# aikiriao/AAD

Hardware: AMD Instinct MI355X
Metric: Msamples/s encode+decode, 48 kHz stereo 4-bit (higher is better)
Workload: dtype int32

## Files before the change

### aad_amd/capi.py

```python
import ctypes as C
import os

import numpy as np


class AADApiResult:
    OK = 0
    INVALID_ARGUMENT = 1
    INVALID_FORMAT = 2
    INSUFFICIENT_BUFFER = 3
    INSUFFICIENT_DATA = 4
    PARAMETER_NOT_SET = 5
    NG = 6
    _names = {0: "OK", 1: "INVALID_ARGUMENT", 2: "INVALID_FORMAT", 3: "INSUFFICIENT_BUFFER",
              4: "INSUFFICIENT_DATA", 5: "PARAMETER_NOT_SET", 6: "NG"}

    @classmethod
    def name(cls, v):
        return cls._names.get(int(v), str(v))


class AADHeaderInfo(C.Structure):
    _fields_ = [("format_version", C.c_uint32), ("codec_version", C.c_uint32),
                ("num_channels", C.c_uint16), ("num_samples", C.c_uint32),
# ... 48 lines not shown

STREAM_DESC_DTYPE = np.dtype([("pcm_offset", "<u8"), ("data_offset", "<u8"), ("data_size", "<u8"),
                              ("num_samples", "<u4"), ("reserved", "<u4")])
ERROR_STATS_DTYPE = np.dtype([("rms_error", "<f8"), ("mean_abs_error", "<f8"), ("max_abs_error", "<f8")])
WINDOW_DTYPE = np.dtype([("stream", "<i8"), ("first_frame", "<i8")])
SAMPLE_INT16, SAMPLE_FLOAT32 = 0, 1
SAMPLE_FLOAT16, SAMPLE_BFLOAT16 = 4, 5
RESAMPLE_NO_BANK = 0xFFFF
WINDOW_GAIN_STORE, WINDOW_GAIN_ADD = 0, 1
RECONSTRUCT_DECODED, RECONSTRUCT_RESIDUAL = 0, 1
OPTION_LANE_MAPPING, OPTION_TRIAL_LANES, OPTION_STAGING_THREADS, OPTION_TILE_KBYTES, OPTION_COMPARE_ORDER = 0, 1, 2, 3, 4
LANE_MAPPINGS = {"auto": 0, "dense": 1, "quad": 2, "quad-fused": 3, "dense-tiled": 4}
TRIAL_LANES = {"dual": 0, "single": 1}
OPTION_SIMD_ROLE = 5
SIMD_ROLE_OFF = -1
LANE_STATE_DTYPE = np.dtype([("weight", "<i4", (4,)), ("history", "<i4", (4,)),
                             ("stepsize_index", "<i4"), ("quantize_error", "<i4")])

_PKG_DIR = os.path.dirname(os.path.abspath(__file__))
LIBRARY_PATH = os.environ.get("AAD_HIP_LIBRARY", os.path.join(_PKG_DIR, "libaad_hip.so"))

LEGACY_SYMBOLS = [
    "AADEncoder_CalculateBlockSize", "AADEncoder_EncodeHeader", "AADEncoder_CalculateWorkSize",
    "AADEncoder_Create", "AADEncoder_Destroy", "AADEncoder_SetEncodeParameter", "AADEncoder_EncodeWhole",
    "AADDecoder_DecodeHeader", "AADDecoder_CalculateWorkSize", "AADDecoder_Create", "AADDecoder_Destroy",
    "AADDecoder_SetHeader", "AADDecoder_DecodeBlock", "AADDecoder_DecodeWhole",
]
HIP_SYMBOLS = [
    "AADHip_GetDeviceCount", "AADHip_ContextCreate", "AADHip_ContextDestroy", "AADHip_ContextSynchronize",
    "AADHip_ContextLastError", "AADHip_ContextSignalNextRun", "AADHip_SignalNextRunSupported", "AADHip_ContextSetOption", "AADHip_CalculateEncodedSize", "AADHip_EncodePlanCreate",
    "AADHip_EncodePlanDestroy", "AADHip_EncodePlanRun", "AADHip_DecodePlanCreate", "AADHip_DecodePlanDestroy",
    "AADHip_DecodePlanRun", "AADHip_EncodeBatch", "AADHip_DecodeBatch",
    "AADHip_ReconstructPlanCreate", "AADHip_ReconstructPlanDestroy", "AADHip_ReconstructPlanRun",
    "AADHip_ReconstructBatch", "AADHip_SegmentedEncodePlanCreate", "AADHip_SegmentedEncodeBatch",
    "AADHip_SegmentedReconstructPlanCreate", "AADHip_SegmentedReconstructBatch",
    "AADHip_WindowDecodePlanCreate", "AADHip_WindowDecodePlanDestroy", "AADHip_WindowDecodePlanRun",
    "AADHip_WindowDecodePlanRunStats", "AADHip_WindowDecodePlanRunGain", "AADHip_WindowDecodePlanRunPlaced", "AADHip_WindowDecodePlanRunPlacedStats",
    "AADHip_MixedWindowDecodePlanCreate", "AADHip_ChannelMixWindowDecodePlanCreate",
    "AADHip_PlanarEncodePlanCreate", "AADHip_PlanarEncodePlanRun",
    "AADHip_PlanarReconstructPlanCreate", "AADHip_PlanarReconstructPlanRun", "AADHip_PlanarReconstructPlanRunStats",
    "AADHip_WindowReconstructPlanCreate", "AADHip_WindowReconstructPlanDestroy", "AADHip_WindowReconstructPlanRun",
    "AADHip_ResamplerCreate", "AADHip_ResamplerDestroy", "AADHip_ResamplerBank", "AADHip_ResamplerSourceFrames",
    "AADHip_ResamplerResolve", "AADHip_ResamplerRun", "AADHip_ResamplerRunGain", "AADHip_ResamplerRunStats",
    "AADHip_ResamplerCreateWide",
]
WAV_SYMBOLS = ["AADWav_ParseHeader", "AADWav_WriteHeader", "AADWav_ConvertToPcm16"]
SYNTH_SYMBOLS = ["AADSynth_Generate"]


class AADWavInfo(C.Structure):
    _fields_ = [("format_tag", C.c_uint16), ("num_channels", C.c_uint16), ("sampling_rate", C.c_uint32),
                ("bits_per_sample", C.c_uint16), ("num_samples", C.c_uint32), ("data_offset", C.c_uint64),
                ("data_size", C.c_uint64)]


def _declare_legacy(lib):
    u8p, i32pp = C.POINTER(C.c_uint8), C.POINTER(C.POINTER(C.c_int32))
    lib.AADEncoder_CalculateBlockSize.argtypes = [C.c_uint16, C.c_uint16, C.c_uint32,
                                                  C.POINTER(C.c_uint16), C.POINTER(C.c_uint32)]
# ... 65 lines not shown
    lib.AADHip_PlanarReconstructPlanRun.restype = C.c_int
    lib.AADHip_PlanarReconstructPlanRunStats.argtypes = [vp, vp, vp, vp, vp, vp]
    lib.AADHip_PlanarReconstructPlanRunStats.restype = C.c_int
    lib.AADHip_WindowReconstructPlanCreate.argtypes = [vp, C.POINTER(AADEncodeParameter), C.POINTER(AADHipPlanarLayout),
                                                       C.POINTER(AADHipSegmentation), C.c_uint32, vp, C.POINTER(vp)]
    lib.AADHip_WindowReconstructPlanCreate.restype = C.c_int
    lib.AADHip_WindowReconstructPlanDestroy.argtypes = [vp]
    lib.AADHip_WindowReconstructPlanDestroy.restype = None
    lib.AADHip_WindowReconstructPlanRun.argtypes = [vp, vp, C.c_uint64, vp, C.c_uint32, C.c_uint64, vp, C.POINTER(AADHipPlanarOutput),
                                                    vp, vp]
    lib.AADHip_WindowReconstructPlanRun.restype = C.c_int
    lib.AADHip_EncodePlanDestroy.argtypes = [vp]
    lib.AADHip_EncodePlanDestroy.restype = None
    lib.AADHip_EncodePlanRun.argtypes = [vp, vp, vp, vp]
    lib.AADHip_EncodePlanRun.restype = C.c_int
    lib.AADHip_DecodePlanCreate.argtypes = [vp, C.POINTER(AADHeaderInfo), C.c_int32, C.c_uint32, vp, C.POINTER(vp)]
    lib.AADHip_DecodePlanCreate.restype = C.c_int
    lib.AADHip_DecodePlanDestroy.argtypes = [vp]
    lib.AADHip_DecodePlanDestroy.restype = None
    lib.AADHip_DecodePlanRun.argtypes = [vp, vp, vp]
    lib.AADHip_DecodePlanRun.restype = C.c_int
    lib.AADHip_WindowDecodePlanCreate.argtypes = [vp, C.POINTER(AADHeaderInfo), C.c_int32, C.c_uint32, vp, C.POINTER(vp)]
    lib.AADHip_WindowDecodePlanCreate.restype = C.c_int
    lib.AADHip_MixedWindowDecodePlanCreate.argtypes = [vp, C.c_uint32, C.c_int32, C.c_uint32, vp, vp, C.POINTER(vp)]
    lib.AADHip_MixedWindowDecodePlanCreate.restype = C.c_int
    lib.AADHip_ChannelMixWindowDecodePlanCreate.argtypes = [vp, C.c_uint32, C.c_int32, C.c_uint32, vp, vp, C.POINTER(vp)]
    lib.AADHip_ChannelMixWindowDecodePlanCreate.restype = C.c_int
    lib.AADHip_WindowDecodePlanDestroy.argtypes = [vp]
    lib.AADHip_WindowDecodePlanDestroy.restype = None
    lib.AADHip_WindowDecodePlanRun.argtypes = [vp, vp, C.c_uint64, vp, C.c_uint32, C.c_int32, vp]
# ... 169 lines not shown
```

### aad_amd/csrc/aad_encode.hip.h

```cpp
#ifndef AAD_ENCODE_HIP_H
#define AAD_ENCODE_HIP_H

#include "aad_device.hip.h"
#include "aad_pcm_convert.h"
#include "aad_segments.h"

namespace aad {

constexpr bool kEncTM = true;

template <int BITS>
__device__ __forceinline__ int32_t index_delta_arith(uint32_t mag)
{
  if (BITS == 4) {
    const uint32_t corr = __builtin_amdgcn_perm(0u, 0x00161514u, mag) & 0xFFu;
    return (int32_t)(2u << mag) - (int32_t)corr;
  } else if (BITS == 3) {
    return mag < 2 ? (int32_t)mag - 16 : (int32_t)(2u << (2u * mag));
  } else {
    return mag ? 40 : -14;
  }
}

template <int BITS>
// ... 1864 lines not shown
  if constexpr (rec_has_stats(REC)) {
    if constexpr (SEG) rec.template finish<true>(a.stats + (uint64_t)a.stats_stream[s] * ch + c, total - warm_end);
    else rec.template finish<false>(a.stats + lane, total > a.lead_frames ? total - a.lead_frames : 0u);
  }

  if (!SEG && a.state_out && writer) {
    LaneStateRecord r;
    r.weight[0] = F.w0; r.weight[1] = F.w1; r.weight[2] = F.w2; r.weight[3] = F.w3;
    r.history[0] = F.h0; r.history[1] = F.h1; r.history[2] = F.h2; r.history[3] = F.h3;
    r.stepsize_index = F.idxb - kIdxBias;
    r.quantize_error = last_qd;
    a.state_out[lane] = r;
  }
}

}

#endif
```

### aad_amd/csrc/aad_encode_launch.hip.h

```cpp
#ifndef AAD_ENCODE_LAUNCH_HIP_H
#define AAD_ENCODE_LAUNCH_HIP_H

#include "aad_encode.hip.h"
#include "aad_launch.h"

namespace aad {

template <int BITS, bool QUAD, bool TRIALS, bool DUAL, bool RING = false, bool SEG = false, int IN = kInInterleaved, int REC = kRecNone>
void launch_encode_mapped(const KernelArgsFor<IN, REC> &a, const EncodeLaunch &p, hipStream_t stream)
{
  const dim3 grid(p.grid), block(p.workgroup);
  if (a.channels == 1) {
    if constexpr (IN != kInPlanarI16)
      AAD_LAUNCH((encode_streams_kernel<BITS, 1, false, QUAD, TRIALS, DUAL, RING, SEG, IN, REC>), grid, block, p.lds, stream, a);
  } else if constexpr (IN == kInInterleaved && REC != kRecNone) {
  } else if (a.channels == 2 && a.mid_side)
    AAD_LAUNCH((encode_streams_kernel<BITS, 2, true, QUAD, TRIALS, DUAL, RING, SEG, IN, REC>), grid, block, p.lds, stream, a);
  else if (a.channels == 2)
    AAD_LAUNCH((encode_streams_kernel<BITS, 2, false, QUAD, TRIALS, DUAL, RING, SEG, IN, REC>), grid, block, p.lds, stream, a);
  else if constexpr (!QUAD && !RING)
    AAD_LAUNCH((encode_streams_kernel<BITS, 0, false, false, TRIALS, false, false, SEG, IN, REC>), grid, block, p.lds, stream, a);
}

template <int BITS, bool SEG, int IN = kInInterleaved, int REC = kRecNone>
// ... 50 lines not shown
    a.stats = r.stats;
    a.stats_stream = r.stats_stream;
  }
  auto by_bits = [&](auto seg) {
    constexpr bool SEG = decltype(seg)::value;
    switch (a.bits) {
      case 4: launch_encode<4, SEG, IN, REC>(a, p, stream); break;
      case 3: launch_encode<3, SEG, IN, REC>(a, p, stream); break;
      default: launch_encode<2, SEG, IN, REC>(a, p, stream); break;
    }
  };
  if (r.chain_table) by_bits(std::true_type{});
  else by_bits(std::false_type{});
}

extern template void launch_encode_run<kInPlanarI16, kRecNone>(const EncodeRun &, const EncodeLaunch &, hipStream_t);
extern template void launch_encode_run<kInPlanarF32, kRecNone>(const EncodeRun &, const EncodeLaunch &, hipStream_t);
#define AAD_EXTERN_REC_RUN(REC)                                                                                    \
  extern template void launch_encode_run<kInInterleaved, REC>(const EncodeRun &, const EncodeLaunch &, hipStream_t); \
  extern template void launch_encode_run<kInPlanarI16, REC>(const EncodeRun &, const EncodeLaunch &, hipStream_t);   \
  extern template void launch_encode_run<kInPlanarF32, REC>(const EncodeRun &, const EncodeLaunch &, hipStream_t);
AAD_EXTERN_REC_RUN(kRecI16)
AAD_EXTERN_REC_RUN(kRecF32)
AAD_EXTERN_REC_RUN(kRecI16Stats)
AAD_EXTERN_REC_RUN(kRecF32Stats)
AAD_EXTERN_REC_RUN(kRecStatsOnly)
#undef AAD_EXTERN_REC_RUN

}

// ... 2 lines not shown
```

### aad_amd/csrc/aad_hip_engine.hip

```cpp
#include <hip/hip_runtime.h>

#include <cstdio>
#include <cstdlib>
#include <cstring>
#include <algorithm>
#include <condition_variable>
#include <functional>
#include <mutex>
#include <new>
#include <thread>
#include <vector>

#include "../../include/aad_hip.h"
#include "aad_compare.hip.h"
#include "aad_launch.h"
#include "aad_decode.hip.h"
#include "aad_decode_window.hip.h"
#include "aad_decode_window_mixed.hip.h"
#include "aad_decode_window_channel_mix.hip.h"
#include "aad_encode.hip.h"
#include "aad_encode_launch.hip.h"
#include "aad_format.h"
#include "aad_hip_internal.h"
#include "aad_resample.hip.h"
#include "aad_tiles.h"
#include "aad_window_reconstruct.hip.h"

namespace aad {
thread_local LaunchSignal tl_launch_signal = {nullptr, nullptr};
}

static_assert(sizeof(AADHipStreamDesc) == sizeof(aad::StreamDesc), "stream table layout");
static_assert(sizeof(AADHipLaneState) == sizeof(aad::LaneStateRecord), "lane state layout");
static_assert(sizeof(AADHipErrorStats) == sizeof(aad::ErrorStatsRecord), "error stats layout");

struct Staging {
  void *host = nullptr, *dev = nullptr;
  size_t cap = 0;
};

struct StagingPool {
  std::vector<std::thread> threads;
  std::mutex lock;
  std::condition_variable work, done;
// ... 48 lines not shown
  AADHipStreamDesc *d_sources;
  uint32_t num_sources;
  uint8_t *d_lanes;
  uint64_t lanes_capacity;
};

struct AADHipEncodePlan {
  AADHipContext *ctx;
  EncodePlanKind kind;
  aad::EncodeRun run;
  void *d_table;
  uint64_t *d_out_base;
  uint32_t *d_stats_stream;
  uint64_t stats_records;
  WindowPlanPart *windows;
};

struct AADHipDecodePlan {
  AADHipContext *ctx;
  aad::DecodeArgs args;
  aad::StreamDesc *d_streams;
  uint64_t *d_prefix;
};

struct AADHipWindowDecodePlan {
  AADHipContext *ctx;
  aad::DecodeArgs args;
  aad::StreamDesc *d_streams;
  bool mixed;
  aad::StreamFormat *d_formats;
// ... 356 lines not shown
  }
  if (output != nullptr && !aad::planar_output_ok(args.channels, num_streams, streams, output)) {
    snprintf(ctx->last_error, sizeof(ctx->last_error),
             "planar reconstruct plan: output rows refused (sample type, reserved, a stride below the rows, or past 64-bit offsets)");
    return AAD_APIRESULT_INVALID_ARGUMENT;
  }
  AADHipEncodePlan *p = new (std::nothrow) AADHipEncodePlan();
  if (p == nullptr) return AAD_APIRESULT_NG;
  p->ctx = ctx;
  p->kind = output != nullptr ? EncodePlanKind::Reconstruct : (layout != nullptr ? EncodePlanKind::Rows : EncodePlanKind::Frames);
  p->d_table = nullptr;
  p->d_out_base = nullptr;
  p->d_stats_stream = nullptr;
  p->windows = nullptr;
  p->stats_records = (uint64_t)num_streams * args.channels;
  DeviceGuard guard(ctx);
  bool ok = guard.ok;
  if (ok && segmentation != nullptr) {
    aad::ChainDesc *d_chains = nullptr;
    ok = upload(ctx, &d_chains, chains.data(), chains.size());
    p->d_table = d_chains;
    use_chain_table(&run, d_chains, (uint32_t)chains.size());
  } else if (ok) {
    aad::StreamDesc *d_streams = nullptr;
    ok = upload(ctx, &d_streams, reinterpret_cast<const aad::StreamDesc *>(streams), num_streams);
    p->d_table = d_streams;
    run.args.streams = d_streams;
  }
  if (ok && output != nullptr) {
    const std::vector<uint64_t> base =
// ... 214 lines not shown
const char *AADHip_ContextLastError(const struct AADHipContext *ctx) { return ctx ? ctx->last_error : ""; }

void AADHipInternal_ContextOptionsFromEnvironment(struct AADHipContext *ctx)
{
  static const char *const kMappings[] = {"auto", "dense", "quad", "quad-fused", "dense-tiled"};
  static const char *const kTrialLanes[] = {"dual", "single"};
  ctx->signal_refused = AADHip_SignalNextRunSupported() == 0;
  ctx->knobs.lane_mapping = option_from_env("AAD_HIP_MAPPING", kMappings, 5);
  ctx->knobs.trial_lanes = option_from_env("AAD_HIP_TRIAL_LANES", kTrialLanes, 2);
  const char *ring = getenv("AAD_HIP_ENCODE_RING"), *enc_pad = getenv("AAD_HIP_ENCODE_LDS_PAD");
  const char *dec_pad = getenv("AAD_HIP_DECODE_LDS_PAD"), *nt_min = getenv("AAD_HIP_DECODE_NT_MIN");
  ctx->knobs.encode_ring = ring != nullptr && ring[0] == '0' ? 0 : (ring != nullptr && ring[0] == '2' ? 2 : 1);
  ctx->knobs.encode_lds_pad = enc_pad ? atoi(enc_pad) : -1;
  ctx->knobs.decode_lds_pad = dec_pad ? atoi(dec_pad) : -1;
  ctx->knobs.decode_nt_min = nt_min ? (uint64_t)atoll(nt_min) : 0ull;
  static const char *const kCompareOrders[] = {"auto", "sequential"};
  ctx->compare_sequential = option_from_env("AAD_HIP_COMPARE_ORDER", kCompareOrders, 2);
  const char *threads = getenv("AAD_HIP_STAGING_THREADS");
  if (threads != nullptr && threads[0] >= '1' && threads[0] <= '8' && threads[1] == '\0') ctx->staging_threads = threads[0] - '0';
  const char *tile = getenv("AAD_HIP_TILE_KBYTES");
  if (tile != nullptr) {
    const long long v = atoll(tile);
    if (v > 0 && v <= 0x7FFFFFFF) ctx->tile_bytes = (int64_t)v << 10;
  }
}

int32_t AADHipInternal_ContextDevice(const struct AADHipContext *ctx) { return ctx->device; }

int32_t AADHip_SignalNextRunSupported(void)
{
// ... 17 lines not shown
AADApiResult AADHip_ContextSetOption(struct AADHipContext *ctx, int32_t option, int32_t value)
{
  if (ctx == nullptr) return AAD_APIRESULT_INVALID_ARGUMENT;
  switch (option) {
    case AAD_HIP_OPTION_LANE_MAPPING:
      if (value < AAD_HIP_LANE_MAPPING_AUTO || value > AAD_HIP_LANE_MAPPING_DENSE_TILED) return AAD_APIRESULT_INVALID_ARGUMENT;
      ctx->knobs.lane_mapping = value;
      return AAD_APIRESULT_OK;
    case AAD_HIP_OPTION_TRIAL_LANES:
      if (value != AAD_HIP_TRIAL_LANES_DUAL && value != AAD_HIP_TRIAL_LANES_SINGLE) return AAD_APIRESULT_INVALID_ARGUMENT;
      ctx->knobs.trial_lanes = value;
      return AAD_APIRESULT_OK;
    case AAD_HIP_OPTION_SIMD_ROLE:
      if (value < AAD_HIP_SIMD_ROLE_OFF || value > AAD_HIP_SIMD_ROLE_3) return AAD_APIRESULT_INVALID_ARGUMENT;
      ctx->knobs.simd_role = value;
      return AAD_APIRESULT_OK;
    case AAD_HIP_OPTION_COMPARE_ORDER:
      if (value != 0 && value != 1) return AAD_APIRESULT_INVALID_ARGUMENT;
      ctx->compare_sequential = value;
      return AAD_APIRESULT_OK;
    case AAD_HIP_OPTION_STAGING_THREADS:
      if (value < 0 || value > 8) return AAD_APIRESULT_INVALID_ARGUMENT;
      ctx->staging_threads = value;
      return AAD_APIRESULT_OK;
    case AAD_HIP_OPTION_TILE_KBYTES:
      if (value < 0) return AAD_APIRESULT_INVALID_ARGUMENT;
      ctx->tile_bytes = (int64_t)value << 10;
      return AAD_APIRESULT_OK;
    default:
      return AAD_APIRESULT_INVALID_ARGUMENT;
// ... 41 lines not shown
AADApiResult AADHip_SegmentedEncodePlanCreate(struct AADHipContext *ctx, const struct AADEncodeParameter *parameter,
                                              const struct AADHipSegmentation *segmentation, uint32_t num_streams,
                                              const struct AADHipStreamDesc *streams, struct AADHipEncodePlan **plan)
{
  if (ctx == nullptr || parameter == nullptr || segmentation == nullptr || plan == nullptr || (num_streams != 0 && streams == nullptr))
    return AAD_APIRESULT_INVALID_ARGUMENT;
  *plan = nullptr;
  if (segmentation->segment_blocks == 0) return AAD_APIRESULT_INVALID_ARGUMENT;
  return encode_plan_create(ctx, parameter, nullptr, nullptr, segmentation, num_streams, streams, plan);
}

AADApiResult AADHip_EncodePlanRun(struct AADHipEncodePlan *plan, const int16_t *device_pcm, uint8_t *device_data,
                                  struct AADHipLaneState *device_state)
{
  return encode_plan_run(plan, EncodePlanKind::Frames, device_pcm, device_data, nullptr, device_state);
}


AADApiResult AADHip_PlanarEncodePlanCreate(struct AADHipContext *ctx, const struct AADEncodeParameter *parameter,
                                           const struct AADHipPlanarLayout *layout, const struct AADHipSegmentation *segmentation,
                                           uint32_t num_streams, const struct AADHipStreamDesc *streams, struct AADHipEncodePlan **plan)
{
  if (ctx == nullptr || parameter == nullptr || layout == nullptr || plan == nullptr || (num_streams != 0 && streams == nullptr))
    return AAD_APIRESULT_INVALID_ARGUMENT;
  *plan = nullptr;
  if (!planar_fields_ok(layout, segmentation)) return AAD_APIRESULT_INVALID_ARGUMENT;
  return encode_plan_create(ctx, parameter, layout, nullptr, segmentation, num_streams, streams, plan);
}

AADApiResult AADHip_PlanarEncodePlanRun(struct AADHipEncodePlan *plan, const void *device_samples, uint8_t *device_data,
// ... 1876 lines not shown
```

### aad_amd/csrc/aad_launch_policy.h

```cpp
#ifndef AAD_LAUNCH_POLICY_H
#define AAD_LAUNCH_POLICY_H

#include <stdint.h>

#include "../../include/aad_hip.h"
#include "aad_lds_layout.h"

namespace aad {

struct Device {
  uint32_t cus, lds_per_cu;
};

struct Knobs {
  int32_t lane_mapping = AAD_HIP_LANE_MAPPING_AUTO;
  int32_t trial_lanes = AAD_HIP_TRIAL_LANES_DUAL;
  int32_t encode_ring = 1;
  int32_t encode_lds_pad = -1;
  int32_t decode_lds_pad = -1;
  uint64_t decode_nt_min = 0;
  int32_t simd_role = AAD_HIP_SIMD_ROLE_OFF;
};

struct EncodeBatch {
  uint32_t bits, channels, streams, trials, block_size;
  bool ring_ok;
};

struct DecodeBatch {
  uint64_t blocks;
  uint32_t streams, channels, bits, samples_per_block, block_size, code_phase_uniform;
  bool pcm_aligned16, pcm_base_aligned16, stream_stores;
};

enum class EncodeKernel { Dense, DenseRing, Quad, QuadDual };
struct EncodeLaunch {
// ... 86 lines not shown
    }
    return p;
  }
  p.kernel = EncodeKernel::Dense;
  uint32_t static_lds = dense_encoder_lds(b.bits, b.channels);
  p.workgroup = dense_encode_workgroup(d, lanes, static_lds);
  p.grid = grid_for(lanes, p.workgroup);
  if (p.trials) return p;
  if (b.ring_ok && b.channels <= 2 && encode_ring_wanted(k, b.bits, b.channels, p.workgroup)) {
    p.kernel = EncodeKernel::DenseRing;
    p.lds = (p.workgroup / 64u) * (uint32_t)(b.channels == 1 ? kLdsRingBytesPerWave<1> : kLdsRingBytesPerWave<2>);
    static_lds = (uint32_t)kLdsCodeStageOff + p.lds;
  }
  if (p.workgroup == 256u) p.lds += dense_encode_lds_pad(d, k, b.bits, lanes, static_lds);
  return p;
}

inline EncodeLaunch plan_reconstruct_encode(const Device &d, const Knobs &k, const EncodeBatch &b)
{
  Knobs r = k;
  r.trial_lanes = AAD_HIP_TRIAL_LANES_SINGLE;
  r.encode_ring = 0;
  return plan_encode(d, r, b);
}

inline bool planar_output_rows_ok(uint32_t channels, uint64_t num_streams, uint64_t longest, const AADHipPlanarOutput *o)
{
  if (o == nullptr || channels == 0) return false;
  if ((o->sample_type != AAD_HIP_SAMPLE_INT16 && o->sample_type != AAD_HIP_SAMPLE_FLOAT32) || o->reserved != 0) return false;
  if (channels > 1 && o->channel_stride < longest) return false;
// ... 297 lines not shown
```

### aad_amd/engine.py

```python
import ctypes as C
from collections import namedtuple

import numpy as np

from .capi import (AADApiResult, AADHeaderInfo, AADHipResampleRatio, RESAMPLE_NO_BANK, AADHipPlanarLayout, AADHipPlanarOutput, AADHipSegmentation, ApiError, ERROR_STATS_DTYPE, LANE_MAPPINGS, LANE_STATE_DTYPE,
                   OPTION_COMPARE_ORDER, OPTION_LANE_MAPPING, OPTION_SIMD_ROLE, OPTION_STAGING_THREADS, OPTION_TILE_KBYTES, OPTION_TRIAL_LANES, RECONSTRUCT_DECODED, RECONSTRUCT_RESIDUAL,
                   SAMPLE_BFLOAT16, SAMPLE_FLOAT16, SAMPLE_FLOAT32, SAMPLE_INT16, SIMD_ROLE_OFF, STREAM_DESC_DTYPE, TRIAL_LANES, WINDOW_DTYPE, WINDOW_GAIN_ADD, WINDOW_GAIN_STORE, load_library, make_parameter)


def _check(where, rc):
    if rc != AADApiResult.OK:
        raise ApiError(where, rc)


def _round_up(v, a):
    return (v + a - 1) // a * a


def tensor_span(t):
    if any(int(s) == 0 for s in t.shape):
        return 0
    return 1 + sum((int(s) - 1) * int(st) for s, st in zip(t.shape, t.stride()))


# ... 159 lines not shown
        _check("AADHip_ContextSetOption",
               self.lib.AADHip_ContextSetOption(self._ctx, OPTION_STAGING_THREADS, int(threads)))

    def set_tile_kbytes(self, kbytes=0):
        _check("AADHip_ContextSetOption",
               self.lib.AADHip_ContextSetOption(self._ctx, OPTION_TILE_KBYTES, int(kbytes)))

    def set_compare_order(self, sequential=False):
        _check("AADHip_ContextSetOption",
               self.lib.AADHip_ContextSetOption(self._ctx, OPTION_COMPARE_ORDER, 1 if sequential else 0))

    def set_simd_role(self, simd=None):
        _check("AADHip_ContextSetOption",
               self.lib.AADHip_ContextSetOption(self._ctx, OPTION_SIMD_ROLE, SIMD_ROLE_OFF if simd is None else int(simd)))

    def synchronize(self):
        _check("AADHip_ContextSynchronize", self.lib.AADHip_ContextSynchronize(self._ctx))

    def encoded_size(self, param, num_samples):
        return int(self.lib.AADHip_CalculateEncodedSize(C.byref(param), num_samples))

    def encode_plan(self, param, descs, segment_blocks=None, warmup_blocks=0):
        descs = np.ascontiguousarray(descs, dtype=STREAM_DESC_DTYPE)
        plan = C.c_void_p()
        if segment_blocks is None:
            _check("AADHip_EncodePlanCreate",
                   self.lib.AADHip_EncodePlanCreate(self._ctx, C.byref(param), len(descs), descs.ctypes.data, C.byref(plan)))
        else:
            seg = AADHipSegmentation(int(segment_blocks), int(warmup_blocks))
            _check("AADHip_SegmentedEncodePlanCreate",
# ... 617 lines not shown
        return self._extents[kind]

    def run(self, pcm, data, state=None, ordered=True):
        if state is not None and self.segmented:
            raise ValueError("a segmented encode plan takes no state")
        e = self.engine
        e.tensor("pcm", pcm, e.torch.int16, self.extent("interleaved"), rows_in_place=True, memo=self._memo)
        e.tensor("data", data, e.torch.uint8, self.extent("images"), rows_in_place=True, memo=self._memo)
        e.state_tensor(state, len(self.descs), self.param.num_channels, self._memo)
        sp = state.data_ptr() if state is not None else None
        cur = self.engine._enter() if ordered else None
        _check("AADHip_EncodePlanRun",
               self.engine.lib.AADHip_EncodePlanRun(self.handle, pcm.data_ptr(), data.data_ptr(), sp))
        if ordered:
            self.engine._exit(cur)

    def close(self):
        if self.handle:
            self.engine.lib.AADHip_EncodePlanDestroy(self.handle)
            self.handle = None

    def __del__(self):
        try:
            self.close()
        except Exception:
            pass


class PlanarEncodePlan(EncodePlan):
    def __init__(self, engine, handle, param, descs, dtype, channel_stride):
# ... 489 lines not shown
        assert enc_engine.stream.cuda_stream != dec_engine.stream.cuda_stream, "the two contexts need streams of their own"
        torch = enc_engine.torch
        self.torch, self.ring, self.k = torch, ring, 0
        self.enc_engine, self.dec_engine = enc_engine, dec_engine
        self._take_simd_roles(_simd_roles.setdefault(enc_engine.device, SimdRoleAllocator()) if simd_roles else None)
        self.enc = enc_engine.uniform_encode_plan(param, streams, samples)
        self.images = [torch.zeros((streams, self.enc.stride), dtype=torch.uint8, device="cuda:%d" % enc_engine.device)
                       for _ in range(ring)]
        zero = torch.zeros((streams, samples, param.num_channels), dtype=torch.int16, device=self.images[0].device)
        self.enc.run(zero, self.images[0])
        torch.cuda.synchronize()
        self.header = parse_header(bytes(self.images[0][0, :31].cpu().numpy()))
        self.dec = dec_engine.uniform_decode_plan(self.header, streams, self.images[0].stride(0), self.enc.image_size)
        self.encoded = [HipEvent() for _ in range(ring)]
        self.decoded = [torch.cuda.Event() for _ in range(ring)]

    def step(self, pcm, out, timing=None):
        k, ring = self.k, self.ring
        self.k += 1
        b = k % ring
        s_enc, s_dec = self.enc_engine.stream, self.dec_engine.stream
        if k >= ring and k % (ring // 2) == 0:
            s_enc.wait_event(self.decoded[(k - ring // 2 - 1) % ring])
        encoded = self.encoded[b] if timing is None else timing[1]
        self.enc_engine.signal_next(encoded, start=None if timing is None else timing[0])
        self.enc.run(pcm, self.images[b], None, ordered=False)
        encoded.wait_on(s_dec)
        if timing is not None:
            self.dec_engine.signal_next(timing[3], start=timing[2])
        self.dec.run(self.images[b], out, ordered=False)
        self.decoded[b].record(s_dec)
        return self.images[b]

    def close(self):
        self.torch.cuda.synchronize()
        self.enc.close()
        self.dec.close()
        for e in self.encoded:
            e.close()
        self._release_simd_roles()

    def _take_simd_roles(self, allocator):
        self._roles = allocator
        self._role_slot = allocator.acquire(self._set_simd_roles) if allocator is not None else None

    def _set_simd_roles(self, enc_simd, dec_simd):
        self.enc_engine.set_simd_role(enc_simd)
        self.dec_engine.set_simd_role(dec_simd)

    def _release_simd_roles(self):
        if getattr(self, "_role_slot", None) is not None:
            self._roles.release(self._role_slot)
            self._role_slot = None


def parse_header(data):
    if len(data) < 31 or data[:4] != b"AAD\x00":
        raise ApiError("parse_header", AADApiResult.INVALID_FORMAT)
    be = lambda o, n: int.from_bytes(data[o:o + n], "big")
    return AADHeaderInfo(format_version=be(4, 4), codec_version=be(8, 4), num_channels=be(12, 2),
                         num_samples=be(14, 4), sampling_rate=be(18, 4), bits_per_sample=be(22, 2),
                         block_size=be(24, 2), num_samples_per_block=be(26, 4), ch_process_method=data[30])

# ... 3 lines not shown
```

### include/aad_hip.h

```cpp
#ifndef AAD_HIP_H_INCLUDED
#define AAD_HIP_H_INCLUDED

#include <stdint.h>
#include "aad.h"
#include "aad_encoder.h"

#define AAD_HIP_MAX_NUM_CHANNELS 8

struct AADHipContext;
struct AADHipEncodePlan;
struct AADHipDecodePlan;

struct AADHipStreamDesc {
  uint64_t pcm_offset;
  uint64_t data_offset;
  uint64_t data_size;
  uint32_t num_samples;
  uint32_t reserved;
};

struct AADHipLaneState {
  int32_t weight[4];
  int32_t history[4];
  int32_t stepsize_index;
// ... 8 lines not shown

AADApiResult AADHip_ContextCreate(int32_t device_index, void *hip_stream, struct AADHipContext **context);
void AADHip_ContextDestroy(struct AADHipContext *context);
AADApiResult AADHip_ContextSynchronize(struct AADHipContext *context);
const char *AADHip_ContextLastError(const struct AADHipContext *context);

AADApiResult AADHip_ContextSignalNextRun(struct AADHipContext *context, void *hip_start_event, void *hip_stop_event);
int32_t AADHip_SignalNextRunSupported(void);

enum AADHipOption {
  AAD_HIP_OPTION_LANE_MAPPING = 0,
  AAD_HIP_OPTION_TRIAL_LANES = 1,
  AAD_HIP_OPTION_STAGING_THREADS = 2,
  AAD_HIP_OPTION_TILE_KBYTES = 3,
  AAD_HIP_OPTION_COMPARE_ORDER = 4,
  AAD_HIP_OPTION_SIMD_ROLE = 5
};
enum AADHipSimdRole {
  AAD_HIP_SIMD_ROLE_OFF = -1,
  AAD_HIP_SIMD_ROLE_0 = 0, AAD_HIP_SIMD_ROLE_1 = 1, AAD_HIP_SIMD_ROLE_2 = 2, AAD_HIP_SIMD_ROLE_3 = 3
};
enum AADHipLaneMapping {
  AAD_HIP_LANE_MAPPING_AUTO = 0,
  AAD_HIP_LANE_MAPPING_DENSE = 1,
  AAD_HIP_LANE_MAPPING_QUAD = 2,
  AAD_HIP_LANE_MAPPING_QUAD_FUSED = 3,
  AAD_HIP_LANE_MAPPING_DENSE_TILED = 4
};
enum AADHipTrialLanes {
  AAD_HIP_TRIAL_LANES_DUAL = 0,
  AAD_HIP_TRIAL_LANES_SINGLE = 1
};
AADApiResult AADHip_ContextSetOption(struct AADHipContext *context, int32_t option, int32_t value);

uint64_t AADHip_CalculateEncodedSize(const struct AADEncodeParameter *parameter, uint32_t num_samples);


AADApiResult AADHip_EncodePlanCreate(
    struct AADHipContext *context, const struct AADEncodeParameter *parameter,
    uint32_t num_streams, const struct AADHipStreamDesc *streams,
    struct AADHipEncodePlan **plan);
void AADHip_EncodePlanDestroy(struct AADHipEncodePlan *plan);

AADApiResult AADHip_EncodePlanRun(
    struct AADHipEncodePlan *plan, const int16_t *device_pcm, uint8_t *device_data,
    struct AADHipLaneState *device_state);


struct AADHipSegmentation {
  uint32_t segment_blocks;
  uint32_t warmup_blocks;
};
AADApiResult AADHip_SegmentedEncodePlanCreate(
    struct AADHipContext *context, const struct AADEncodeParameter *parameter,
    const struct AADHipSegmentation *segmentation,
    uint32_t num_streams, const struct AADHipStreamDesc *streams,
    struct AADHipEncodePlan **plan);


AADApiResult AADHip_DecodePlanCreate(
    struct AADHipContext *context, const struct AADHeaderInfo *format, int32_t has_file_header,
// ... 251 lines not shown
```

Measured before the change: 122,100.

## Split pipeline encode into resumable spans so decode overlaps encode tail

Adds a span-encode kernel that resumes from saved lane state at chunk-aligned frames. The encode+decode pipeline now encodes the first ~95% of frames, signals the decoder's stream, then encodes the remainder on the decoder's stream (roles off by default). The intent is to let the decoder's stream start earlier and shorten the cross-stream dependency. It adds a second launch, state records that must be zeroed each ring half, and extra synchronisation when the split is first enabled.

```diff
diff --git a/aad_amd/capi.py b/aad_amd/capi.py
--- a/aad_amd/capi.py
+++ b/aad_amd/capi.py
@@ -86,6 +86,7 @@
 TRIAL_LANES = {"dual": 0, "single": 1}
 OPTION_SIMD_ROLE = 5
 SIMD_ROLE_OFF = -1
+OPTION_PIPELINE_SPLIT = 6
 LANE_STATE_DTYPE = np.dtype([("weight", "<i4", (4,)), ("history", "<i4", (4,)),
                              ("stepsize_index", "<i4"), ("quantize_error", "<i4")])
 
@@ -115,6 +116,7 @@
     "AADHip_ResamplerCreate", "AADHip_ResamplerDestroy", "AADHip_ResamplerBank", "AADHip_ResamplerSourceFrames",
     "AADHip_ResamplerResolve", "AADHip_ResamplerRun", "AADHip_ResamplerRunGain", "AADHip_ResamplerRunStats",
     "AADHip_ResamplerCreateWide",
+    "AADHip_EncodePlanRunSpan", "AADHip_EncodePlanSpanSupported", "AADHip_EncodePlanSpanFloor", "AADHip_EncodePlanPipelineSplit",
 ]
 WAV_SYMBOLS = ["AADWav_ParseHeader", "AADWav_WriteHeader", "AADWav_ConvertToPcm16"]
 SYNTH_SYMBOLS = ["AADSynth_Generate"]
@@ -210,6 +212,14 @@
     lib.AADHip_EncodePlanDestroy.restype = None
     lib.AADHip_EncodePlanRun.argtypes = [vp, vp, vp, vp]
     lib.AADHip_EncodePlanRun.restype = C.c_int
+    lib.AADHip_EncodePlanRunSpan.argtypes = [vp, vp, vp, vp, C.c_uint32, C.c_uint32]
+    lib.AADHip_EncodePlanRunSpan.restype = C.c_int
+    lib.AADHip_EncodePlanSpanSupported.argtypes = [vp]
+    lib.AADHip_EncodePlanSpanSupported.restype = C.c_int32
+    lib.AADHip_EncodePlanSpanFloor.argtypes = [vp, C.c_uint32]
+    lib.AADHip_EncodePlanSpanFloor.restype = C.c_uint32
+    lib.AADHip_EncodePlanPipelineSplit.argtypes = [vp, C.c_int32]
+    lib.AADHip_EncodePlanPipelineSplit.restype = C.c_uint32
     lib.AADHip_DecodePlanCreate.argtypes = [vp, C.POINTER(AADHeaderInfo), C.c_int32, C.c_uint32, vp, C.POINTER(vp)]
     lib.AADHip_DecodePlanCreate.restype = C.c_int
     lib.AADHip_DecodePlanDestroy.argtypes = [vp]
diff --git a/aad_amd/csrc/aad_encode.hip.h b/aad_amd/csrc/aad_encode.hip.h
--- a/aad_amd/csrc/aad_encode.hip.h
+++ b/aad_amd/csrc/aad_encode.hip.h
@@ -2,6 +2,7 @@
 #define AAD_ENCODE_HIP_H
 
 #include "aad_device.hip.h"
+#include "aad_encode_span.h"
 #include "aad_pcm_convert.h"
 #include "aad_segments.h"
 
@@ -1902,6 +1903,85 @@
   }
 }
 
+
+struct SpanEncodeArgs : EncodeArgs {
+  uint32_t first_frame, frame_count;
+};
+static_assert(kSpanSeedFrames == (uint32_t)kTaps && kSpanChunkFrames == (uint32_t)kChunk, "aad_encode_span.h counts in the kernels' units");
+
+template <int BITS, int CHF, bool MS>
+__global__ void __launch_bounds__(256) encode_span_kernel(SpanEncodeArgs a)
+{
+  static_assert(CHF == 1 || CHF == 2, "the quad mapping: mono / stereo");
+  __shared__ __attribute__((aligned(16))) char lds[kLdsBytesEncoderStatic<BITS, CHF, true, false>];
+  __shared__ uint32_t s_wave_simd[4];
+  if (a.simd_role) publish_wave_simd(s_wave_simd);
+  stage_tables<BITS, true, kWideStepShift, true>(lds);
+  uint64_t thread = (uint64_t)blockIdx.x * blockDim.x + threadIdx.x;
+  if (a.simd_role) {
+    if ((threadIdx.x >> 6) != elected_worker_wave(a.simd_role - 1u, s_wave_simd)) return;
+    thread = (uint64_t)blockIdx.x * 64u + (threadIdx.x & 63u);
+  }
+  constexpr uint32_t ch = CHF;
+  const uint64_t lane = (thread >> 6) * 16u + quad_slot<kEncTM>();
+  const uint32_t tap = quad_tap<kEncTM>();
+  const bool writer = tap == 0;
+  if (lane >= (uint64_t)a.num_streams * ch) return;
+  const uint32_t s = (uint32_t)(lane / ch), c = (uint32_t)(lane % ch);
+  const StreamDesc sd = a.uni.enabled ? uniform_stream(a.uni, s) : a.streams[s];
+  const SampleSource<MS, kInInterleaved> src = {a.pcm + sd.pcm_offset, ch, c, sd.num_samples};
+  uint8_t *out = a.data + sd.data_offset;
+  const uint32_t total = sd.num_samples, spb = a.samples_per_block;
+  const uint64_t begin = a.first_frame, end = begin + a.frame_count;
+
+  Lane F = {0, 0, 0, 0, 0, 0, 0, 0, kIdxBias};
+  int32_t last_qd = 0;
+  if (a.state) {
+    const LaneStateRecord r = a.state[lane];
+    F = {r.weight[0], r.weight[1], r.weight[2], r.weight[3],
+         r.history[0], r.history[1], r.history[2], r.history[3],
+         min(max(r.stepsize_index, 0), (int32_t)AAD_STEP_INDEX_MAX) + kIdxBias};
+    last_qd = r.quantize_error;
+  }
+  if (c == 0 && writer && begin == 0) {
+    const uint32_t *t = reinterpret_cast<const uint32_t *>(a.header_template);
+#pragma unroll
+    for (int i = 0; i < 7; i++) {
+      uint32_t d = t[i];
+      if (i == 3) d = (d & 0x0000FFFFu) | ((total >> 24) << 16) | (((total >> 16) & 0xFFu) << 24);
+      if (i == 4) d = (d & 0xFFFF0000u) | ((total >> 8) & 0xFFu) | ((total & 0xFFu) << 8);
+      reinterpret_cast<U32 *>(out + 4 * i)->v = d;
+    }
+    reinterpret_cast<U16 *>(out + 28)->v = (uint16_t)t[7];
+    out[30] = (uint8_t)(t[7] >> 16);
+  }
+
+  uint64_t first = begin / spb * spb;
+  uint64_t block_off = kFileHeaderBytes + begin / spb * a.block_size;
+  for (; first < end; first += spb, block_off += a.block_size) {
+    const uint32_t n = total - first < spb ? (uint32_t)(total - first) : spb;
+    const uint32_t stop = end - first < n ? (uint32_t)(end - first) : n;
+    const uint32_t skip = begin > first ? (uint32_t)(begin - first) - kTaps : 0u;
+    if (begin <= first) {
+      seed_history(F, src, first, n);
+      (void)write_block_header(F, out + block_off + (uint64_t)c * kBlockHeaderBytesPerCh, writer);
+    }
+    uint8_t *body = out + block_off + (uint64_t)kBlockHeaderBytesPerCh * ch + (uint64_t)(skip / kChunk) * Pack<BITS>::kChunkBytes * ch;
+    QuadLane L = to_quad(F, tap);
+    (void)run_block<BITS, CHF, MS, true, kPassEncode>(L, src, first + skip, stop - skip, ch, c, writer, body, lds, last_qd);
+    F = from_quad<kEncTM>(L);
+  }
+
+  if (a.state_out && writer) {
+    LaneStateRecord r;
+    r.weight[0] = F.w0; r.weight[1] = F.w1; r.weight[2] = F.w2; r.weight[3] = F.w3;
+    r.history[0] = F.h0; r.history[1] = F.h1; r.history[2] = F.h2; r.history[3] = F.h3;
+    r.stepsize_index = F.idxb - kIdxBias;
+    r.quantize_error = last_qd;
+    a.state_out[lane] = r;
+  }
+}
+
 }
 
 #endif
diff --git a/aad_amd/csrc/aad_encode_launch.hip.h b/aad_amd/csrc/aad_encode_launch.hip.h
--- a/aad_amd/csrc/aad_encode_launch.hip.h
+++ b/aad_amd/csrc/aad_encode_launch.hip.h
@@ -88,6 +88,8 @@
   else by_bits(std::false_type{});
 }
 
+void launch_encode_span(const SpanEncodeArgs &a, const EncodeLaunch &p, hipStream_t stream);
+
 extern template void launch_encode_run<kInPlanarI16, kRecNone>(const EncodeRun &, const EncodeLaunch &, hipStream_t);
 extern template void launch_encode_run<kInPlanarF32, kRecNone>(const EncodeRun &, const EncodeLaunch &, hipStream_t);
 #define AAD_EXTERN_REC_RUN(REC)                                                                                    \
diff --git a/aad_amd/csrc/aad_encode_span.h b/aad_amd/csrc/aad_encode_span.h
--- /dev/null
+++ b/aad_amd/csrc/aad_encode_span.h
@@ -0,0 +1,26 @@
+#ifndef AAD_ENCODE_SPAN_H
+#define AAD_ENCODE_SPAN_H
+
+#include <stdint.h>
+
+namespace aad {
+
+constexpr uint32_t kSpanSeedFrames = 4, kSpanChunkFrames = 16;
+
+inline uint32_t span_floor(uint32_t total, uint32_t spb, uint32_t want)
+{
+  if (want >= total || spb == 0) return total;
+  const uint32_t first = want / spb * spb;
+  const uint32_t n = total - first < spb ? total - first : spb;
+  const uint32_t in = want - first;
+  if (n < kSpanSeedFrames || in < kSpanSeedFrames) return first;
+  const uint32_t chunks = (n - kSpanSeedFrames) / kSpanChunkFrames;
+  const uint32_t k = (in - kSpanSeedFrames) / kSpanChunkFrames;
+  return first + kSpanSeedFrames + kSpanChunkFrames * (k < chunks ? k : chunks);
+}
+
+inline bool span_resumable(uint32_t total, uint32_t spb, uint32_t frame) { return frame <= total && span_floor(total, spb, frame) == frame; }
+
+}
+
+#endif
diff --git a/aad_amd/csrc/aad_hip_engine.hip b/aad_amd/csrc/aad_hip_engine.hip
--- a/aad_amd/csrc/aad_hip_engine.hip
+++ b/aad_amd/csrc/aad_hip_engine.hip
@@ -28,6 +28,22 @@
 
 namespace aad {
 thread_local LaunchSignal tl_launch_signal = {nullptr, nullptr};
+
+void launch_encode_span(const SpanEncodeArgs &a, const EncodeLaunch &p, hipStream_t stream)
+{
+  const dim3 grid(p.grid), block(p.workgroup);
+  auto by_channels = [&](auto bits) {
+    constexpr int BITS = decltype(bits)::value;
+    if (a.channels == 1) AAD_LAUNCH((encode_span_kernel<BITS, 1, false>), grid, block, 0, stream, a);
+    else if (a.mid_side) AAD_LAUNCH((encode_span_kernel<BITS, 2, true>), grid, block, 0, stream, a);
+    else AAD_LAUNCH((encode_span_kernel<BITS, 2, false>), grid, block, 0, stream, a);
+  };
+  switch (a.bits) {
+    case 4: by_channels(std::integral_constant<int, 4>{}); break;
+    case 3: by_channels(std::integral_constant<int, 3>{}); break;
+    default: by_channels(std::integral_constant<int, 2>{}); break;
+  }
+}
 }
 
 static_assert(sizeof(AADHipStreamDesc) == sizeof(aad::StreamDesc), "stream table layout");
@@ -106,6 +122,8 @@
   uint32_t *d_stats_stream;
   uint64_t stats_records;
   WindowPlanPart *windows;
+  bool equal_length;
+  uint32_t span_frames;
 };
 
 struct AADHipDecodePlan {
@@ -492,6 +510,9 @@
   p->d_stats_stream = nullptr;
   p->windows = nullptr;
   p->stats_records = (uint64_t)num_streams * args.channels;
+  p->span_frames = num_streams != 0 ? streams[0].num_samples : 0;
+  p->equal_length = num_streams != 0;
+  for (uint32_t i = 1; i < num_streams; i++) p->equal_length = p->equal_length && streams[i].num_samples == p->span_frames;
   DeviceGuard guard(ctx);
   bool ok = guard.ok;
   if (ok && segmentation != nullptr) {
@@ -736,6 +757,8 @@
   ctx->knobs.encode_lds_pad = enc_pad ? atoi(enc_pad) : -1;
   ctx->knobs.decode_lds_pad = dec_pad ? atoi(dec_pad) : -1;
   ctx->knobs.decode_nt_min = nt_min ? (uint64_t)atoll(nt_min) : 0ull;
+  const char *split = getenv("AAD_HIP_PIPELINE_SPLIT");
+  ctx->knobs.pipeline_split = split != nullptr && atoi(split) >= 1 && atoi(split) <= 1000 ? atoi(split) : -1;
   static const char *const kCompareOrders[] = {"auto", "sequential"};
   ctx->compare_sequential = option_from_env("AAD_HIP_COMPARE_ORDER", kCompareOrders, 2);
   const char *threads = getenv("AAD_HIP_STAGING_THREADS");
@@ -783,6 +806,10 @@
     case AAD_HIP_OPTION_SIMD_ROLE:
       if (value < AAD_HIP_SIMD_ROLE_OFF || value > AAD_HIP_SIMD_ROLE_3) return AAD_APIRESULT_INVALID_ARGUMENT;
       ctx->knobs.simd_role = value;
+      return AAD_APIRESULT_OK;
+    case AAD_HIP_OPTION_PIPELINE_SPLIT:
+      if (value < -1 || value == 0 || value > 1000) return AAD_APIRESULT_INVALID_ARGUMENT;
+      ctx->knobs.pipeline_split = value;
       return AAD_APIRESULT_OK;
     case AAD_HIP_OPTION_COMPARE_ORDER:
       if (value != 0 && value != 1) return AAD_APIRESULT_INVALID_ARGUMENT;
@@ -854,6 +881,82 @@
                                   struct AADHipLaneState *device_state)
 {
   return encode_plan_run(plan, EncodePlanKind::Frames, device_pcm, device_data, nullptr, device_state);
+}
+
+
+namespace {
+const char *span_refusal(const AADHipEncodePlan *plan, aad::EncodeLaunch *launch)
+{
+  const aad::EncodeRun &r = plan->run;
+  if (plan->kind != EncodePlanKind::Frames || r.chain_table || r.in != aad::kInInterleaved || r.rec != aad::kRecNone)
+    return "interleaved int16 frames of an unsegmented encode plan are needed";
+  if (!plan->equal_length) return "streams of equal length are needed";
+  if (r.args.trials != 0 || r.args.lead_frames != 0) return "a plan without trial search is needed";
+  if (r.args.channels > 2 || r.args.bits < 2 || r.args.bits > 4) return "mono or stereo streams of 2 to 4 bits are needed";
+  const aad::EncodeBatch batch{r.args.bits, r.args.channels, r.args.num_streams, 0, r.args.block_size, false};
+  *launch = aad::plan_encode(plan->ctx->device_info, plan->ctx->knobs, batch);
+  if (launch->kernel != aad::EncodeKernel::Quad) return "a batch that takes the quad lane mapping is needed";
+  return nullptr;
+}
+}
+
+int32_t AADHip_EncodePlanSpanSupported(const struct AADHipEncodePlan *plan)
+{
+  aad::EncodeLaunch launch;
+  return plan != nullptr && span_refusal(plan, &launch) == nullptr ? 1 : 0;
+}
+
+uint32_t AADHip_EncodePlanSpanFloor(const struct AADHipEncodePlan *plan, uint32_t frame)
+{
+  if (plan == nullptr || !plan->equal_length) return 0;
+  return aad::span_floor(plan->span_frames, plan->run.args.samples_per_block, frame);
+}
+
+uint32_t AADHip_EncodePlanPipelineSplit(const struct AADHipEncodePlan *plan, int32_t roles_in_force)
+{
+  if (plan == nullptr || !plan->equal_length) return 0;
+  return aad::plan_pipeline_split(plan->ctx->knobs, roles_in_force != 0, plan->span_frames, plan->run.args.samples_per_block);
+}
+
+AADApiResult AADHip_EncodePlanRunSpan(struct AADHipEncodePlan *plan, const int16_t *device_pcm, uint8_t *device_data,
+                                      struct AADHipLaneState *device_state, uint32_t first_frame, uint32_t frame_count)
+{
+  if (plan == nullptr || device_pcm == nullptr || device_data == nullptr) return AAD_APIRESULT_INVALID_ARGUMENT;
+  AADHipContext *ctx = plan->ctx;
+  const aad::LaunchSignal signal = take_signal(ctx);
+  DeviceGuard guard(ctx);
+  if (!guard.ok) return AAD_APIRESULT_NG;
+  auto refuse = [&](const char *why) {
+    snprintf(ctx->last_error, sizeof(ctx->last_error), "AADHip_EncodePlanRunSpan: %s", why);
+    return finish_signal(ctx, signal, AAD_APIRESULT_INVALID_ARGUMENT);
+  };
+  aad::EncodeLaunch launch;
+  if (const char *why = span_refusal(plan, &launch)) return refuse(why);
+  const uint32_t total = plan->span_frames, spb = plan->run.args.samples_per_block;
+  if (first_frame > total || frame_count > total - first_frame) return refuse("the span reaches past the streams' end");
+  const uint32_t last = first_frame + frame_count;
+  if (!aad::span_resumable(total, spb, first_frame) || !aad::span_resumable(total, spb, last))
+    return refuse("both ends of a span must be resumable frames (AADHip_EncodePlanSpanFloor)");
+  if (device_state == nullptr && (first_frame != 0 || last != total))
+    return refuse("device_state is needed: only a span from frame 0 to the streams' end runs without one");
+  if (frame_count == 0) {
+    aad::tl_launch_signal = signal;
+    return finish_signal(ctx, signal, AAD_APIRESULT_OK);
+  }
+  aad::SpanEncodeArgs a;
+  static_cast<aad::EncodeArgs &>(a) = plan->run.args;
+  a.pcm = device_pcm;
+  a.data = device_data;
+  a.state = reinterpret_cast<const aad::LaneStateRecord *>(device_state);
+  a.state_out = reinterpret_cast<aad::LaneStateRecord *>(device_state);
+  a.trial_scratch = nullptr;
+  a.trial_slot_bytes = 0;
+  a.simd_role = launch.simd_role;
+  a.first_frame = first_frame;
+  a.frame_count = frame_count;
+  aad::tl_launch_signal = signal;
+  aad::launch_encode_span(a, launch, ctx->stream);
+  return finish_signal(ctx, signal, hip_ok(ctx, hipGetLastError(), "encode span launch") ? AAD_APIRESULT_OK : AAD_APIRESULT_NG);
 }
 
 
diff --git a/aad_amd/csrc/aad_launch_policy.h b/aad_amd/csrc/aad_launch_policy.h
--- a/aad_amd/csrc/aad_launch_policy.h
+++ b/aad_amd/csrc/aad_launch_policy.h
@@ -4,6 +4,7 @@
 #include <stdint.h>
 
 #include "../../include/aad_hip.h"
+#include "aad_encode_span.h"
 #include "aad_lds_layout.h"
 
 namespace aad {
@@ -20,6 +21,7 @@
   int32_t decode_lds_pad = -1;
   uint64_t decode_nt_min = 0;
   int32_t simd_role = AAD_HIP_SIMD_ROLE_OFF;
+  int32_t pipeline_split = -1;
 };
 
 struct EncodeBatch {
@@ -136,6 +138,14 @@
   }
   if (p.workgroup == 256u) p.lds += dense_encode_lds_pad(d, k, b.bits, lanes, static_lds);
   return p;
+}
+
+constexpr int32_t kPipelineSplitRoles = 1000, kPipelineSplitAlone = 950;
+inline uint32_t plan_pipeline_split(const Knobs &k, bool roles_in_force, uint32_t total, uint32_t spb)
+{
+  const int32_t permille = k.pipeline_split >= 1 ? k.pipeline_split : (roles_in_force ? kPipelineSplitRoles : kPipelineSplitAlone);
+  if (permille >= 1000) return total;
+  return span_floor(total, spb, (uint32_t)((uint64_t)total * (uint32_t)permille / 1000u));
 }
 
 inline EncodeLaunch plan_reconstruct_encode(const Device &d, const Knobs &k, const EncodeBatch &b)
diff --git a/aad_amd/engine.py b/aad_amd/engine.py
--- a/aad_amd/engine.py
+++ b/aad_amd/engine.py
@@ -4,7 +4,7 @@
 import numpy as np
 
 from .capi import (AADApiResult, AADHeaderInfo, AADHipResampleRatio, RESAMPLE_NO_BANK, AADHipPlanarLayout, AADHipPlanarOutput, AADHipSegmentation, ApiError, ERROR_STATS_DTYPE, LANE_MAPPINGS, LANE_STATE_DTYPE,
-                   OPTION_COMPARE_ORDER, OPTION_LANE_MAPPING, OPTION_SIMD_ROLE, OPTION_STAGING_THREADS, OPTION_TILE_KBYTES, OPTION_TRIAL_LANES, RECONSTRUCT_DECODED, RECONSTRUCT_RESIDUAL,
+                   OPTION_COMPARE_ORDER, OPTION_LANE_MAPPING, OPTION_PIPELINE_SPLIT, OPTION_SIMD_ROLE, OPTION_STAGING_THREADS, OPTION_TILE_KBYTES, OPTION_TRIAL_LANES, RECONSTRUCT_DECODED, RECONSTRUCT_RESIDUAL,
                    SAMPLE_BFLOAT16, SAMPLE_FLOAT16, SAMPLE_FLOAT32, SAMPLE_INT16, SIMD_ROLE_OFF, STREAM_DESC_DTYPE, TRIAL_LANES, WINDOW_DTYPE, WINDOW_GAIN_ADD, WINDOW_GAIN_STORE, load_library, make_parameter)
 
 
@@ -197,6 +197,10 @@
         _check("AADHip_ContextSetOption",
                self.lib.AADHip_ContextSetOption(self._ctx, OPTION_SIMD_ROLE, SIMD_ROLE_OFF if simd is None else int(simd)))
 
+    def set_pipeline_split(self, permille=None):
+        _check("AADHip_ContextSetOption",
+               self.lib.AADHip_ContextSetOption(self._ctx, OPTION_PIPELINE_SPLIT, -1 if permille is None else int(permille)))
+
     def synchronize(self):
         _check("AADHip_ContextSynchronize", self.lib.AADHip_ContextSynchronize(self._ctx))
 
@@ -844,6 +848,27 @@
                self.engine.lib.AADHip_EncodePlanRun(self.handle, pcm.data_ptr(), data.data_ptr(), sp))
         if ordered:
             self.engine._exit(cur)
+
+    def span_supported(self):
+        return bool(self.engine.lib.AADHip_EncodePlanSpanSupported(self.handle))
+
+    def span_floor(self, frame):
+        return int(self.engine.lib.AADHip_EncodePlanSpanFloor(self.handle, int(frame)))
+
+    def pipeline_split(self, roles_in_force):
+        return int(self.engine.lib.AADHip_EncodePlanPipelineSplit(self.handle, 1 if roles_in_force else 0))
+
+    def run_span(self, pcm, data, state, first_frame, frame_count, ordered=True):
+        e = self.engine
+        e.tensor("pcm", pcm, e.torch.int16, self.extent("interleaved"), rows_in_place=True, memo=self._memo)
+        e.tensor("data", data, e.torch.uint8, self.extent("images"), rows_in_place=True, memo=self._memo)
+        e.state_tensor(state, len(self.descs), self.param.num_channels, self._memo)
+        sp = state.data_ptr() if state is not None else None
+        cur = self.engine._enter() if ordered else None
+        rc = self.engine.lib.AADHip_EncodePlanRunSpan(self.handle, pcm.data_ptr(), data.data_ptr(), sp, int(first_frame), int(frame_count))
+        if ordered:
+            self.engine._exit(cur)
+        _check("AADHip_EncodePlanRunSpan", rc)
 
     def close(self):
         if self.handle:
@@ -1363,6 +1388,21 @@
         self.dec = dec_engine.uniform_decode_plan(self.header, streams, self.images[0].stride(0), self.enc.image_size)
         self.encoded = [HipEvent() for _ in range(ring)]
         self.decoded = [torch.cuda.Event() for _ in range(ring)]
+        self.samples = samples
+        self.enc2 = dec_engine.uniform_encode_plan(param, streams, samples)
+        self.states = None
+        if self.enc.span_supported() and self.enc2.span_supported():
+            self.states = torch.zeros((ring, streams * param.num_channels, 10), dtype=torch.int32, device=self.images[0].device)
+        self._plan_split()
+
+    def _plan_split(self):
+        cut = self.enc.pipeline_split(self._roles_in_force) if self.states is not None else self.samples
+        cut = cut if 0 < cut < self.samples else None
+        if cut is not None and self.k and getattr(self, "cut", None) is None:
+            self.torch.cuda.synchronize()
+            self.states.zero_()
+            self.torch.cuda.synchronize()
+        self.cut = cut
 
     def step(self, pcm, out, timing=None):
         k, ring = self.k, self.ring
@@ -1371,10 +1411,23 @@
         s_enc, s_dec = self.enc_engine.stream, self.dec_engine.stream
         if k >= ring and k % (ring // 2) == 0:
             s_enc.wait_event(self.decoded[(k - ring // 2 - 1) % ring])
-        encoded = self.encoded[b] if timing is None else timing[1]
-        self.enc_engine.signal_next(encoded, start=None if timing is None else timing[0])
-        self.enc.run(pcm, self.images[b], None, ordered=False)
-        encoded.wait_on(s_dec)
+        if self.cut is None:
+            encoded = self.encoded[b] if timing is None else timing[1]
+            self.enc_engine.signal_next(encoded, start=None if timing is None else timing[0])
+            self.enc.run(pcm, self.images[b], None, ordered=False)
+            encoded.wait_on(s_dec)
+        else:
+            half = ring // 2
+            if k >= ring and k % half == 0:
+                with self.torch.cuda.stream(s_enc):
+                    self.states[b:b + half].zero_()
+            state, encoded = self.states[b], self.encoded[b]
+            self.enc_engine.signal_next(encoded, start=None if timing is None else timing[0])
+            self.enc.run_span(pcm, self.images[b], state, 0, self.cut, ordered=False)
+            encoded.wait_on(s_dec)
+            if timing is not None:
+                self.dec_engine.signal_next(timing[1])
+            self.enc2.run_span(pcm, self.images[b], state, self.cut, self.samples - self.cut, ordered=False)
         if timing is not None:
             self.dec_engine.signal_next(timing[3], start=timing[2])
         self.dec.run(self.images[b], out, ordered=False)
@@ -1384,18 +1437,22 @@
     def close(self):
         self.torch.cuda.synchronize()
         self.enc.close()
+        self.enc2.close()
         self.dec.close()
         for e in self.encoded:
             e.close()
         self._release_simd_roles()
 
     def _take_simd_roles(self, allocator):
-        self._roles = allocator
+        self._roles, self._roles_in_force = allocator, False
         self._role_slot = allocator.acquire(self._set_simd_roles) if allocator is not None else None
 
     def _set_simd_roles(self, enc_simd, dec_simd):
         self.enc_engine.set_simd_role(enc_simd)
         self.dec_engine.set_simd_role(dec_simd)
+        self._roles_in_force = enc_simd is not None
+        if hasattr(self, "states"):
+            self._plan_split()
 
     def _release_simd_roles(self):
         if getattr(self, "_role_slot", None) is not None:
diff --git a/include/aad_hip.h b/include/aad_hip.h
--- a/include/aad_hip.h
+++ b/include/aad_hip.h
@@ -46,7 +46,8 @@
   AAD_HIP_OPTION_STAGING_THREADS = 2,
   AAD_HIP_OPTION_TILE_KBYTES = 3,
   AAD_HIP_OPTION_COMPARE_ORDER = 4,
-  AAD_HIP_OPTION_SIMD_ROLE = 5
+  AAD_HIP_OPTION_SIMD_ROLE = 5,
+  AAD_HIP_OPTION_PIPELINE_SPLIT = 6
 };
 enum AADHipSimdRole {
   AAD_HIP_SIMD_ROLE_OFF = -1,
@@ -77,6 +78,14 @@
 AADApiResult AADHip_EncodePlanRun(
     struct AADHipEncodePlan *plan, const int16_t *device_pcm, uint8_t *device_data,
     struct AADHipLaneState *device_state);
+
+
+int32_t AADHip_EncodePlanSpanSupported(const struct AADHipEncodePlan *plan);
+uint32_t AADHip_EncodePlanSpanFloor(const struct AADHipEncodePlan *plan, uint32_t frame);
+uint32_t AADHip_EncodePlanPipelineSplit(const struct AADHipEncodePlan *plan, int32_t roles_in_force);
+AADApiResult AADHip_EncodePlanRunSpan(
+    struct AADHipEncodePlan *plan, const int16_t *device_pcm, uint8_t *device_data,
+    struct AADHipLaneState *device_state, uint32_t first_frame, uint32_t frame_count);
 
 
 struct AADHipSegmentation {
```

New measurement: 122,200, median of 2. No clear change (+0.1%).
